# bbuchfink/diamond

Hardware: AMD Instinct MI355X
Metric: GCUPS + aligned queries/s, blastp --fast, 10000 queries vs 1000000-seq DB (seed stage + banded SW extension) (higher is better)
Workload: dtype int16

## Files before the change

### diamond_amd/csrc/ctx.h

```cpp
#pragma once
#include "tuning.h"
#include <hip/hip_runtime.h>
#include <chrono>
#include <cstdio>
#include <cstdlib>
#include <stdint.h>
#include <string>
#include <vector>
#include "../../include/diamond_hip.h"
#include "evalue.h"
#include "seed_ref_state.h"

namespace dmnd {

int fail(int code, const std::string& msg);

#define HIP_TRY(expr)                                                                                     \
	do {                                                                                                  \
		hipError_t e_ = (expr);                                                                           \
		if (e_ != hipSuccess)                                                                             \
			return ::dmnd::fail(DMND_E_DEVICE, std::string(#expr) + ": " + hipGetErrorString(e_));        \
	} while (0)

inline bool spin_sync()
// ... 121 lines not shown
	dmnd::DevBuf mask_lr, mask_pb, mask_scale, mask_pos, mask_ids, mask_soff, mask_long_ids, mask_long_soff, mask_long_pb, mask_long_scale;
	dmnd::DevBuf soft[2], motif_hit, motif_table;
	bool soft_valid[2] = { false, false };
	std::vector<uint64_t> motifs;
	bool own_motifs = false;
	double mask_ms = 0.0;
	double seed_ms[5] = { 0, 0, 0, 0, 0 };
	std::vector<dmnd::DevBuf> keep_trace;
	std::vector<dmnd_ctx*> aux;
	int8_t* pinned_cbs = nullptr; size_t pinned_cbs_cap = 0;
	double ext_stats[12] = { 0 };
	double ext_plan_stats[3] = { 0, 0, 0 };
	double host_ms[3] = { 0, 0, 0 };
	int comp_based_stats = 1;
	int query_contexts = 1;
	int max_target_seqs = 25;
	int frame_shift = 0;
	bool range_culling = false;
	double range_cover = 50.0;
	int fs_channels = 16;
	int max_hsps = 1;
	int global_ranking = 0;
	dmnd::DevBuf alt_targets;
	double top_percent = -1.0;
	double min_id = 0, query_cover = 0, subject_cover = 0, min_bit_score = 0;
	double approx_id = 0;
	dmnd_same_title_fn same_title = nullptr;
	void* same_title_user = nullptr;
	bool reuse_query_index = false;
	uint64_t query_generation = 0;
	uint64_t target_generation = 0;
	dmnd::SeedRefState seed_ref;
	int64_t seed_last_joined = -1;
	dmnd::DevBuf seed_ref_codes, seed_ref_lists, seed_ref_counts;
	void release_seed_ref_buffers() { seed_ref_codes.release(); seed_ref_lists.release(); seed_ref_counts.release(); }
	void release_seed_ref() { release_seed_ref_buffers(); seed_ref.seen = 0; seed_ref.key.clear(); }
	uint64_t cbs_generation = ~(uint64_t)0;
	std::string qindex_signature;
	std::vector<int32_t> source_lens;
	dmnd::DevBuf ext_source_lens;
	uint64_t source_lens_generation = ~(uint64_t)0;
	int ext_mode = -1;
	int band_mode_fast = 1;
	std::vector<unsigned long long> seed_trace;
	double ranking_block_letters = 2e9;
	dmnd::DevBuf seg_tables, seg_cls, seg_work, seg_handed, seg_ranges;
	bool seg_tables_ready = false;
	std::vector<int32_t> seg_last;
	bool seg_last_sorted = true;
	double seg_stats[4] = { 0, 0, 0, 0 };
};

struct KeptTrace {
	int arena = -1;
	bool kept = false;
	std::vector<int64_t> trace_off;
	std::vector<int32_t> P;
	std::vector<int32_t> score, end_i, end_j;
};
int dmnd_swipe_keep(dmnd_ctx* work, const dmnd_ctx* blocks, const dmnd_dp_target* items, int64_t n, int arena, dmnd_hsp* out, KeptTrace& kt);
int dmnd_traceback_kept(dmnd_ctx* work, const dmnd_ctx* blocks, const dmnd_dp_target* items, const KeptTrace& kt, const int64_t* src, int64_t n, dmnd_hsp* out);
namespace dmnd { struct SwipeEnd; }
namespace dmnd { int64_t sweep_rows_min_items(); }
int dmnd_sweep_classes(dmnd_ctx* work, const dmnd_ctx* blocks, const dmnd_dp_target* d_items, const uint32_t* class_count, const uint32_t* class_max_steps, int n_classes,
	const int32_t* order_dev, const int64_t* off_slot_dev, const int32_t* pairs_dev, const int64_t* off_item_dev, uint8_t* trace_dev, dmnd::SwipeEnd* ends_dev);
int dmnd_swipe_shared(dmnd_ctx* work, const dmnd_ctx* blocks, const dmnd_dp_target* items, int64_t n, int mode, uint32_t hsp_values,
	dmnd_hsp* out, uint8_t* transcript, int64_t transcript_cap, int64_t* transcript_used);
int dmnd_swipe_targets(dmnd_ctx* work, const dmnd_ctx* blocks, const int8_t* t, int64_t t_len, const dmnd_dp_target* items, int64_t n, int mode, uint32_t hsp_values,
// ... 13 lines not shown
```

### diamond_amd/csrc/seed_api.hip

```cpp
#include <hip/hip_runtime.h>
#include <algorithm>
#include <cstdlib>
#include <cmath>
#include <cstdio>
#include <cstring>
#include <string>
#include <sys/mman.h>
#include <thread>
#include <vector>
#include <chrono>
#include "ctx.h"
#include "seed_core.h"
#include "seed_kernels.h"

using namespace dmnd;

enum { SEED_CLASSES_LONG_DEFAULT = 1 };

static_assert(sizeof(dmnd_seed_params) == sizeof(SeedParams), "dmnd_seed_params must mirror dmnd::SeedParams");
static_assert(sizeof(dmnd_seed_hit) == 24, "dmnd_seed_hit layout");

extern "C" int dmnd_seed_params_fast(dmnd_seed_params* p, int threads)
{
	if (!p || threads < 1) return fail(DMND_E_ARG, "dmnd_seed_params_fast: bad argument");
// ... 541 lines not shown
		a.matched_count = c->counters.as<unsigned long long>() + sid;
		a.matched_cap = matched_cap;
		a.deferred = nullptr; a.deferred_count = c->counters.as<unsigned long long>() + S + 1; a.deferred_cap = 0;
		a.survivors = nullptr; a.survivor_count = c->counters.as<unsigned long long>() + S + 3; a.survivor_cap = 0;
		a.scored = nullptr; a.scored_count = c->counters.as<unsigned long long>() + S + 4;
		a.need_bits = c->seed_need.as<uint32_t>();
		a.e_key = nullptr; a.e_count = c->counters.as<unsigned long long>() + S + 2; a.e_n = 0;
		a.matrix = c->matrix.as<int8_t>();
		a.hits = c->seed_hits.as<dmnd_seed_hit>(); a.hit_count = c->counters.as<unsigned long long>() + S; a.hit_cap = 0;
		a.fused = fused ? 1 : 0;
		a.level2 = sp.shape_weight[sid] >= 10 ? 1 : 0;
		a.qfold = fused ? c->seed_qfold.as<uint8_t>() : nullptr;
		a.tfold = fused ? c->seed_tfold.as<uint8_t>() : nullptr;
		return a;
	};

	Timer tm(st);
	for (int i = 0; i < 5; ++i) c->seed_ms[i] = 0;
	lap("clears and query ids enqueued");
	SeedRefUse ref_use = SEED_REF_NONE;
	int slice_bits = -1;
	const int64_t ref_windows = seed_ref_windows(t_begin, t_end);
	{
		const int force = [] { const char* e = getenv("DMND_SEED_SLICES"); return e ? (atoi(e) != 0 ? 1 : 0) : -1; }();
		const uint64_t budget = [] { const char* e = getenv("DMND_SEED_SLICES_BUDGET_MB"); return (uint64_t)std::max<long long>(0, e ? atoll(e) : tuning().seed_slices_budget_mb); }() << 20;
		const int64_t min_letters = [] { const char* e = getenv("DMND_SEED_SLICES_MIN_LETTERS"); return e ? atoll(e) : tuning().seed_slices_min_letters; }();
		const uint32_t max_words = [] { const char* e = getenv("DMND_SEED_SLICE_WORDS"); return (uint32_t)std::min<long long>(SEED_SLICE_MAX_WORDS, std::max<long long>(64, e ? atoll(e) : SEED_SLICE_MAX_WORDS)); }();
		slice_bits = seed_slice_bits(bm1_words, slot_bits, max_words);
		const bool sparse_filter = (uint64_t)nq_pos * 4 <= bm1_words * 32;
		const bool eligible = !fused && !classes && nibble_shapes && sp.seed_encoding == SEED_SPACED && slice_bits >= 0 && ref_windows < ((int64_t)1 << 31)
			&& (force == 1 || (t_end - t_begin >= min_letters && sparse_filter && c->seed_last_joined <= tuning().seed_slices_max_joined));
		const int8_t* tseed = c->soft_valid[DMND_TARGET] ? c->soft[DMND_TARGET].as<int8_t>() : c->block[DMND_TARGET].as<int8_t>();
		bool drop = false;
		ref_use = seed_ref_decide(c->seed_ref, seed_ref_key_of(c->target_generation, tseed, t_begin, t_end, sp, slice_bits), force, eligible, seed_ref_cache_bytes(t_begin, t_end, S), budget, &drop);
		if (drop) c->release_seed_ref_buffers();
		if (ref_use == SEED_REF_BUILT) {
			const int64_t n_groups = seed_code_groups(t_begin, t_end);
			DevBuf route[2];
			auto exact = [](DevBuf& b, size_t bytes) {
				if (b.cap == bytes && b.own) return true;
				b.release();
				if (hipMalloc(&b.p, bytes) != hipSuccess) { b.p = nullptr; (void)hipGetLastError(); return false; }
				b.cap = bytes;
				return true;
			};
			bool ok = exact(c->seed_ref_codes, (size_t)n_groups * sizeof(uint64_t)) && c->seed_tflags.ensure((size_t)n_groups * sizeof(uint32_t)) == DMND_OK
				&& exact(c->seed_ref_lists, (size_t)S * (size_t)ref_windows * sizeof(uint32_t)) && exact(c->seed_ref_counts, (size_t)S * 64 * sizeof(uint32_t))
				&& exact(route[0], (size_t)ref_windows) && exact(route[1], (size_t)ref_windows);
			if (ok) {
				tm.start();
				hipError_t e = launch_seed_codes(sp, tseed, t_begin, t_end, c->seed_ref_codes.as<uint64_t>(), c->seed_tflags.as<uint32_t>(), nullptr, st);
				for (int sid = 0; sid < S && e == hipSuccess; ++sid)
					e = launch_seed_route(sp, sid, c->seed_ref_codes.as<uint64_t>(), c->seed_tflags.as<uint32_t>(), t_begin, t_end, slice_bits, route[0].as<uint8_t>(), route[1].as<uint8_t>(),
						c->seed_ref_lists.as<uint32_t>() + (size_t)sid * (size_t)ref_windows, c->seed_ref_counts.as<uint32_t>() + (size_t)sid * 64, &c->sort_tmp, &c->sort_tmp_bytes, st);
				tm.stop(c->seed_ms[0]);
				if (e == hipSuccess) e = sync_stream(st);
				if (e != hipSuccess) { route[0].release(); route[1].release(); c->release_seed_ref(); HIP_TRY(e); }
			}
			route[0].release(); route[1].release();
			seed_ref_built(c->seed_ref, ok);
			if (!ok) { c->release_seed_ref(); ref_use = SEED_REF_NONE; }
			lap("reference cache built");
		}
	}
	auto stream_shape = [&](const SeedArgs& a, int sid) -> hipError_t {
		if (ref_use == SEED_REF_NONE) return launch_seed_stream(a, sid, st);
		return launch_seed_stream_slices(a, sid, c->seed_ref_codes.as<uint64_t>(), c->seed_ref_lists.as<uint32_t>() + (size_t)sid * (size_t)ref_windows,
			c->seed_ref_counts.as<uint32_t>() + (size_t)sid * 64, slice_bits, st);
	};
	auto query_side = [&](const SeedArgs& a, int sid, bool build) -> int {
		if (build) {
			HIP_TRY(launch_seed_build(a, sid, c->seed_qlist.as<uint32_t>() + (size_t)(sid % SB) * nq_pos, c->seed_next.as<uint32_t>(), c->seed_qkeys.as<uint32_t>(),
				&c->sort_tmp, &c->sort_tmp_bytes, st));
		}
		else HIP_TRY(launch_seed_reset(a, sid, st));
		return DMND_OK;
	};
	if (c->soft_valid[DMND_QUERY]) {
		SeedArgs a = args_for(0, 0, 0);
		HIP_TRY(launch_seed_soft_time(a, st));
	}
	std::vector<unsigned long long> counts((size_t)S + 1, 0);
	unsigned long long n_pairs = 0;
	bool hits_done = false;
	char path[128] = "host";
	if (fused) {
		unsigned long long* ctr = c->counters.as<unsigned long long>();
		int64_t m_cap = seed_cap("DMND_SEED_MATCHED_CAP", std::max<int64_t>(std::max<int64_t>((int64_t)1 << 22, 4 * nq_pos), (int64_t)(std::min(c->matched_loc.cap / sizeof(int64_t), c->matched_slot.cap / sizeof(uint32_t)))));
		int64_t surv_cap = seed_cap("DMND_SEED_SURVIVOR_CAP", std::max<int64_t>((int64_t)1 << 20, (int64_t)(c->seed_survivors.cap / sizeof(SeedSurvivor))));
		int64_t hit_cap = seed_cap("DMND_SEED_HIT_CAP", std::max<int64_t>((int64_t)1 << 20, (int64_t)(c->seed_hits.cap / sizeof(dmnd_seed_hit))));
		if (int rc = c->seed_hits.ensure((size_t)hit_cap * sizeof(dmnd_seed_hit))) return rc;
		c->seed_trace.assign((size_t)2 * S, 0);
		int64_t hits_bound = 0;
		std::vector<unsigned long long> host_ctr((size_t)S + 4);
		hipStream_t sb = st;
		Timer tmb(sb);
		unsigned long long hits_seen = 0;
		bool hits_fresh = false;
		auto stage2 = [&](SeedArgs a, int sid, unsigned long long n, unsigned long long ns) -> int {
			HIP_TRY(hipSetDevice(c->device));
			if (hits_bound + (int64_t)ns > hit_cap) {
// ... 365 lines not shown
		if (int rc = c->sort_keys[1].ensure((size_t)n * sizeof(uint64_t))) return rc;
		if (int rc = c->sort_idx[0].ensure((size_t)n * sizeof(uint32_t))) return rc;
		if (int rc = c->sort_idx[1].ensure((size_t)n * sizeof(uint32_t))) return rc;
		uint64_t* keys[2] = { c->sort_keys[0].as<uint64_t>(), c->sort_keys[1].as<uint64_t>() };
		uint32_t* idx[2] = { c->sort_idx[0].as<uint32_t>(), c->sort_idx[1].as<uint32_t>() };
		auto bits_of = [](uint64_t v) { int b = 1; while (b < 64 && (v >> b) != 0) ++b; return b; };
		const std::vector<int64_t>& qlim = c->limits[DMND_QUERY];
		if (c->max_query_len_generation != c->query_generation || c->max_query_len <= 0) {
			int64_t m = 1;
			for (size_t i = 0; i + 1 < qlim.size(); ++i) m = std::max(m, qlim[i + 1] - qlim[i]);
			c->max_query_len = m; c->max_query_len_generation = c->query_generation;
		}
		HIP_TRY(sort_seed_hits(c->seed_hits.as<dmnd_seed_hit>(), c->seed_hits_sorted.as<dmnd_seed_hit>(), n, keys, idx, &c->sort_tmp, &c->sort_tmp_bytes, st,
			bits_of((uint64_t)std::max<size_t>(qlim.size(), 2) - 1), bits_of((uint64_t)c->block_len[DMND_TARGET]), bits_of((uint64_t)c->max_query_len), !sp.use_ungapped));
		HIP_TRY(sync_stream(st));
	}
	lap("hits sorted");
	if (phases) {
		unsigned long long t[8];
		HIP_TRY(copy_now(c->stream, t, c->counters.as<unsigned long long>() + S + 8, sizeof(t), hipMemcpyDeviceToHost));
		std::fprintf(stderr, "SEED_PHASES (ms of workgroup time, summed): start %.1f | windows %.1f | level 1 %.1f | table %.1f | light lists %.1f | heavy lists %.1f\n",
			t[0] / 1e5, t[1] / 1e5, t[2] / 1e5, t[3] / 1e5, t[4] / 1e5, t[5] / 1e5);
	}
	tm.collect();
	c->seed_ms[4] = c->seed_ms[0] + c->seed_ms[1] + c->seed_ms[2] + c->seed_ms[3];
	if (getenv("DMND_TRACE")) {
		std::fprintf(stderr, "dmnd_seed_search: %d shapes, %lld query positions, joined reference positions per shape:", S, (long long)nq_pos);
		for (int sid = 0; sid < S; ++sid) std::fprintf(stderr, " %llu", counts[sid]);
		std::fprintf(stderr, " | pairs %llu | Hamming survivors:", n_pairs);
		for (int sid = 0; sid < S && (size_t)sid < c->seed_trace.size(); ++sid) std::fprintf(stderr, " %llu", c->seed_trace[sid]);
		std::fprintf(stderr, " | deferred:");
		for (int sid = 0; sid < S && (size_t)(S + sid) < c->seed_trace.size(); ++sid) std::fprintf(stderr, " %llu", c->seed_trace[S + sid]);
		std::fprintf(stderr, " | hits %lld | ms index %.2f stream %.2f mask %.2f pairs %.2f | path: %s\n", (long long)c->n_seed_hits, c->seed_ms[0], c->seed_ms[1], c->seed_ms[2], c->seed_ms[3], path);
		const size_t held = c->seed_ref_codes.cap + c->seed_ref_lists.cap + c->seed_ref_counts.cap;
		if (ref_use == SEED_REF_NONE) std::fprintf(stderr, "dmnd_seed_search: stream: plain, reference cache: none, %zu bytes held\n", held);
		else std::fprintf(stderr, "dmnd_seed_search: stream: slices (%d x %g KB), reference cache: %s, %zu bytes held\n", 1 << slice_bits, (double)(bm1_words >> slice_bits) * 4 / 1024, ref_use == SEED_REF_BUILT ? "built" : "kept", held);
	}
	*n_hits = c->n_seed_hits;
	c->seed_last_hits = c->n_seed_hits;
	c->seed_last_joined = 0;
	for (int sid = 0; sid < S; ++sid) c->seed_last_joined += (int64_t)counts[sid];
	return DMND_OK;
}

extern "C" int64_t dmnd_seed_hit_count(const dmnd_ctx* c) { return c ? c->n_seed_hits : -1; }

extern "C" int dmnd_set_seed_hits_resident(dmnd_ctx* c, int on)
{
	if (!c) return fail(DMND_E_ARG, "dmnd_set_seed_hits_resident: ctx is NULL");
	c->seed_hits_stay = on != 0;
	return DMND_OK;
}

extern "C" int dmnd_seed_hits(dmnd_ctx* c, dmnd_seed_hit* out, int64_t cap)
{
	if (!c || (!out && c->n_seed_hits > 0)) return fail(DMND_E_ARG, "dmnd_seed_hits: NULL argument");
	if (cap < c->n_seed_hits) return fail(DMND_E_CAP, "dmnd_seed_hits: buffer too small");
	if (c->n_seed_hits == 0) return DMND_OK;
	if (c->seed_ret_hits == c->n_seed_hits && c->seed_ret_h.p) {
		std::memcpy(out, c->seed_ret_h.as<char>() + c->seed_ret_bytes_header, (size_t)c->n_seed_hits * sizeof(dmnd_seed_hit));
		return DMND_OK;
	}
	HIP_TRY(hipSetDevice(c->device));
	if (int rc = download_bytes(c, out, c->seed_hits_sorted.p, (size_t)c->n_seed_hits * sizeof(dmnd_seed_hit))) return rc;
	return DMND_OK;
}
```

### diamond_amd/csrc/seed_kernels.h

```cpp
#pragma once
#include <hip/hip_runtime.h>
#include <stdint.h>
#include "../../include/diamond_hip.h"
#include "seed_core.h"
#include "seed_chain.h"
#include "seed_slices_core.h"

namespace dmnd {

static const uint64_t SEED_EMPTY = ~0ull;
static const uint32_t LIST_END = 0xffffffffu;
enum : uint32_t { SLOT_JOINED = 1, SLOT_ERASED = 2, SLOT_LOWC = 8 };

struct SeedSlot { uint64_t key; uint32_t head; uint32_t flags; };

struct SeedDeferred { int64_t sloc; uint32_t slot, x; int32_t score, pad; };

struct SeedSurvivor { uint32_t slot, x; int64_t sloc; };

struct SeedScored { uint32_t slot, x; int64_t sloc; int32_t score, chunk; };

struct SeedArgs {
	SeedParams params;
	const int8_t* qdata; const int8_t* tdata;
// ... 26 lines not shown
	uint32_t* matched_slot; int64_t* matched_loc; unsigned long long* matched_count; int64_t matched_cap;
	SeedDeferred* deferred; unsigned long long* deferred_count; int64_t deferred_cap;
	SeedSurvivor* survivors; unsigned long long* survivor_count; int64_t survivor_cap;
	SeedScored* scored; unsigned long long* scored_count;
	uint32_t* need_bits;
	uint64_t* e_key; unsigned long long* e_count; int64_t e_n;
	const int8_t* matrix;
	dmnd_seed_hit* hits; unsigned long long* hit_count; int64_t hit_cap;
	const uint8_t* qfold;
	const uint8_t* tfold;
	int level2;
	int fused;
};

struct SeedClear {
	void* p[8]; uint64_t bytes[8]; uint32_t value[8];
	int n = 0;
	void add(void* ptr, uint64_t nbytes, uint32_t byte_value) { if (ptr && nbytes && n < 8) { p[n] = ptr; bytes[n] = nbytes; value[n] = byte_value; ++n; } }
};
hipError_t launch_seed_clear(const SeedClear& z, hipStream_t st);
hipError_t launch_seed_qid(const int64_t* limits, int64_t n_seqs, uint32_t* qid_of, hipStream_t st);
enum { SEED_NEED_FOLD_WORDS = 8192 };
hipError_t launch_seed_soft_time(const SeedArgs& a, hipStream_t st);
inline int64_t seed_build_work_words(int64_t n) { return 5 * n + 66; }
hipError_t launch_seed_build(const SeedArgs& a, int sid, uint32_t* qlist_out, uint32_t* work, uint32_t* sorted_top, void** tmp, size_t* tmp_bytes, hipStream_t st);
hipError_t launch_seed_reset(const SeedArgs& a, int sid, hipStream_t st);
hipError_t launch_seed_fold(const int8_t* data, int64_t n, uint8_t* out, hipStream_t st);
inline int64_t seed_code_groups(int64_t t_begin, int64_t t_end) { return (t_end - (t_begin & ~(int64_t)15) + 15) / 16 + 2; }
hipError_t launch_seed_codes(const SeedParams& c, const int8_t* tseed, int64_t t_begin, int64_t t_end, uint64_t* codes, uint32_t* flags, uint64_t* planes, hipStream_t st);
hipError_t launch_seed_stream(const SeedArgs& a, int sid, hipStream_t st, bool fused = false);
bool seed_stream_can_fuse(const SeedParams& c);
hipError_t launch_seed_route(const SeedParams& c, int sid, const uint64_t* codes, const uint32_t* flags, int64_t t_begin, int64_t t_end, int slice_bits,
	uint8_t* route, uint8_t* route_sorted, uint32_t* list, uint32_t* counts, void** tmp, size_t* tmp_bytes, hipStream_t st);
hipError_t launch_seed_stream_slices(const SeedArgs& a, int sid, const uint64_t* codes, const uint32_t* list, const uint32_t* counts, int slice_bits, hipStream_t st);
hipError_t launch_seed_mask(const SeedArgs& a, int sid, hipStream_t st, int64_t n_matched = -1);
hipError_t launch_seed_pairs(const SeedArgs& a, int sid, int64_t n_matched, hipStream_t st);
hipError_t launch_seed_pairs_tiled(const SeedArgs& a, int sid, int64_t n_matched, hipStream_t st);
hipError_t launch_seed_count_pairs(const SeedArgs& a, int64_t n_matched, unsigned long long* out, hipStream_t st);
hipError_t launch_seed_post(const SeedArgs& a, int sid, int64_t n_survivors, hipStream_t st, bool clear_scored = true);
hipError_t sort_matched_by_slot(const uint32_t* slot_in, uint32_t* slot_out, const int64_t* loc_in, int64_t* loc_out, int64_t n, int slot_bits,
	void** tmp, size_t* tmp_bytes, hipStream_t st);
hipError_t launch_seed_collect(const SeedArgs& a, int64_t n_matched, hipStream_t st);
hipError_t launch_seed_deferred(const SeedArgs& a, int sid, int64_t n_deferred, hipStream_t st);
hipError_t sort_keys_u64(const uint64_t* in, uint64_t* out, int64_t n, void** tmp, size_t* tmp_bytes, hipStream_t st);
hipError_t sort_seed_hits(const dmnd_seed_hit* hits, dmnd_seed_hit* out, int64_t n, uint64_t* keys[2], uint32_t* idx[2],
	void** tmp, size_t* tmp_bytes, hipStream_t st, int query_bits, int subject_bits, int off_bits, bool equal_scores = false);

struct SeedChain {
	unsigned long long* ctr;
	int S;
	int64_t matched_cap, survivor_cap, hit_cap, tiled_from;
};
hipError_t launch_seed_chain_streamed(const SeedChain& ch, int sid, hipStream_t st);
hipError_t launch_seed_chain_mask(const SeedArgs& a, const SeedChain& ch, int sid, hipStream_t st);
hipError_t launch_seed_chain_shape(const SeedArgs& a, const SeedChain& ch, int sid, hipStream_t st);
inline bool sort_seed_hits_one_key(int query_bits, int subject_bits, int off_bits) { return off_bits >= 1 && off_bits <= 24 && query_bits + subject_bits + off_bits <= 64; }
hipError_t launch_seed_chain_sort(const SeedChain& ch, bool sorted, const dmnd_seed_hit* hits, dmnd_seed_hit* out, int64_t sort_cap, uint64_t* keys[2], uint32_t* idx[2],
	void** tmp, size_t* tmp_bytes, hipStream_t st, int query_bits, int subject_bits, int off_bits, bool equal_scores, char* ret, int64_t ret_hits);

}
```

### diamond_amd/csrc/seed_kernels.hip

```cpp
#include <hip/hip_runtime.h>
#include <stdint.h>
#include "seed_core.h"
#include <algorithm>
#include <cstdlib>
#include <cstring>
#include <cstdio>
#include <rocprim/device/device_radix_sort.hpp>
#include <rocprim/iterator/counting_iterator.hpp>
#include <rocprim/iterator/transform_iterator.hpp>
#include <rocprim/iterator/transform_output_iterator.hpp>
#include <rocprim/device/device_scan.hpp>
#include "seed_kernels.h"

namespace dmnd {

struct SeedClearArgs { char* p[8]; uint64_t bytes[8]; uint64_t first_chunk[9]; uint32_t word[8]; int n; };
__global__ __launch_bounds__(256) void seed_clear_kernel(SeedClearArgs z)
{
	const uint64_t t = (uint64_t)blockIdx.x * blockDim.x + threadIdx.x;
	if (t >= z.first_chunk[8]) return;
	char* base = z.p[0];
	uint64_t bytes = z.bytes[0], first = 0;
	uint32_t w = z.word[0];
#pragma unroll
// ... 669 lines not shown
		}
		__syncthreads();
		PHASE_MARK(4);
		const unsigned n_heavy = hv_n < HEAVY ? hv_n : HEAVY;
		for (unsigned h = 0; h < n_heavy; ++h) {
			const unsigned k = hv_k[h];
			uint32_t count = st_count[k];
			if (count == 0xffffu) count = a.slot(st_slot[k]).flags >> 8;
			filter_list(st_slot[k], st_head[k], count, wg_base + st_loc[k], threadIdx.x, 256);
		}
		__syncthreads();
		PHASE_MARK(5);
		const unsigned n_sv = sv_n < SURV ? sv_n : SURV;
		if (n_sv) {
			if (threadIdx.x == 0) st_base = atomicAdd(a.survivor_count, (unsigned long long)n_sv);
			__syncthreads();
			for (unsigned k = threadIdx.x; k < n_sv; k += blockDim.x) {
				const unsigned long long idx = st_base + k;
				if (idx < (unsigned long long)a.survivor_cap) a.survivors[idx] = SeedSurvivor{ sv_slot[k], sv_x[k], wg_base + sv_loc[k] };
			}
			__syncthreads();
		}
	}
	const unsigned n_staged = st_n < STAGE ? st_n : STAGE;
	if (n_staged == 0) return;
	if (threadIdx.x == 0) st_base = atomicAdd(a.matched_count, (unsigned long long)n_staged);
	__syncthreads();
	for (unsigned k = threadIdx.x; k < n_staged; k += blockDim.x) {
		const unsigned long long idx = st_base + k;
		if (idx < (unsigned long long)a.matched_cap) { a.matched_slot[idx] = st_slot[k]; a.matched_loc[idx] = wg_base + st_loc[k]; }
	}
}

enum { SEED_SLICE_THREADS = 1024, SEED_SLICE_BATCH = 4, SEED_SLICE_QUEUE = 128, SEED_SLICE_STAGE = 32 };
__global__ __launch_bounds__(SEED_SLICE_THREADS) void seed_stream_slices_kernel(SeedArgs a, int64_t base, uint64_t care64, const uint64_t* __restrict__ codes,
	const uint32_t* __restrict__ list, const uint32_t* __restrict__ counts, int slice_bits, uint32_t slice_words)
{
	constexpr int B = SEED_SLICE_BATCH;
	constexpr unsigned WAVES = SEED_SLICE_THREADS / 64, QW = SEED_SLICE_QUEUE, ST = SEED_SLICE_STAGE;
	static_assert(QW >= 128, "a wavefront queues up to 63 + 64 positives before it probes 64");
	__shared__ uint32_t slice[SEED_SLICE_MAX_WORDS];
	__shared__ uint64_t q_key[WAVES][QW];
	__shared__ uint32_t q_off[WAVES][QW];
	__shared__ uint32_t st_slot[WAVES][ST], st_off[WAVES][ST];
	const unsigned s = blockIdx.x & ((1u << slice_bits) - 1), share = blockIdx.x >> slice_bits, shares = gridDim.x >> slice_bits;
	uint64_t begin = 0;
	for (unsigned i = 0; i < s; ++i) begin += counts[i];
	const uint64_t count = counts[s];
	const uint64_t lo = begin + count * share / shares, hi = begin + count * (share + 1) / shares;
	const uint32_t word0 = s * slice_words;
	for (uint32_t i = threadIdx.x; i < slice_words; i += blockDim.x) slice[i] = a.bitmap1[word0 + i];
	__syncthreads();
	const unsigned wave = threadIdx.x >> 6, lane = threadIdx.x & 63u;
	unsigned qn = 0, sn = 0;
	auto rank_in = [&](unsigned long long ballot) { return (unsigned)__builtin_amdgcn_mbcnt_hi((uint32_t)(ballot >> 32), __builtin_amdgcn_mbcnt_lo((uint32_t)ballot, 0u)); };
	auto wave_sync = [&]() { __builtin_amdgcn_fence(__ATOMIC_RELEASE, "wavefront"); __builtin_amdgcn_wave_barrier(); __builtin_amdgcn_fence(__ATOMIC_ACQUIRE, "wavefront"); };
	auto flush = [&]() {
		const unsigned n = sn < ST ? sn : ST;
		unsigned long long at = 0;
		if (lane == 0) at = atomicAdd(a.matched_count, (unsigned long long)n);
		at = ((unsigned long long)(uint32_t)__shfl((int)(at >> 32), 0) << 32) | (uint32_t)__shfl((int)(uint32_t)at, 0);
		wave_sync();
		if (lane < n && at + lane < (unsigned long long)a.matched_cap) { a.matched_slot[at + lane] = st_slot[wave][lane]; a.matched_loc[at + lane] = base + st_off[wave][lane]; }
		wave_sync();
		sn = 0;
	};
	auto probe = [&](bool active, uint64_t seed, uint32_t off) {
		bool found = false;
		uint64_t slot = 0;
		if (active) {
			const uint64_t hh = seed_hash(seed);
			if (!a.level2 || ((a.bitmap[a.bm2_index((uint32_t)hh, seed)] >> (uint32_t)(hh >> 59)) & 1u)) {
				slot = a.home(hh, seed);
				SeedSlot sl = a.slot(slot);
				uint32_t fl = 0;
				for (;;) {
					if (sl.key == SEED_EMPTY) break;
					if (sl.key == seed) { found = true; fl = sl.flags; break; }
					slot = (slot + 1) & a.slot_mask;
					sl = a.slot(slot);
				}
				if (found && !(fl & SLOT_JOINED)) a.slot(slot).flags = fl | SLOT_JOINED;
			}
		}
		const unsigned long long jb = __ballot(found);
		if (jb == 0) return;
		const unsigned k = sn + rank_in(jb);
		if (found) {
			if (k < ST) { st_slot[wave][k] = (uint32_t)slot; st_off[wave][k] = off; }
			else {
				const unsigned long long idx = atomicAdd(a.matched_count, 1ull);
				if (idx < (unsigned long long)a.matched_cap) { a.matched_slot[idx] = (uint32_t)slot; a.matched_loc[idx] = base + off; }
			}
		}
		sn += (unsigned)__builtin_popcountll(jb);
		if (sn >= ST / 2) flush();
	};
	const uint64_t stride = (uint64_t)B * blockDim.x;
	auto entries = [&](uint64_t k0, uint32_t* o) {
#pragma unroll
		for (int j = 0; j < B; ++j) {
			const uint64_t k = k0 + (uint64_t)j * blockDim.x + threadIdx.x;
			o[j] = k < hi ? list[k] : 0xffffffffu;
		}
	};
	auto nibbles = [&](const uint32_t* o, uint64_t* c0, uint64_t* c1) {
#pragma unroll
		for (int j = 0; j < B; ++j) {
			const uint32_t g = o[j] == 0xffffffffu ? 0u : o[j] >> 4;
			c0[j] = codes[g]; c1[j] = codes[g + 1];
		}
	};
	uint32_t off[B], off1[B], off2[B];
	uint64_t c0[B], c1[B], n0[B], n1[B];
	entries(lo, off);
	entries(lo + stride, off1);
	nibbles(off, c0, c1);
	for (uint64_t k0 = lo; k0 < hi; k0 += stride) {
		entries(k0 + 2 * stride, off2);
		nibbles(off1, n0, n1);
#pragma unroll
		for (int j = 0; j < B; ++j) {
			const int sh = (int)(off[j] & 15u) * 4;
			const uint64_t key = (sh == 0 ? c0[j] : (c0[j] >> sh) | (c1[j] << (64 - sh))) & care64;
			const uint32_t h = seed_hash_a(key);
			const uint32_t lw = a.bm1_index(h, key) - word0;
			const uint32_t bw = slice[lw < slice_words ? lw : 0u], need = bm1_bits(h, a.bitmap1_k3);
			const bool pass = off[j] != 0xffffffffu && (bw & need) == need;
			const unsigned long long pb = __ballot(pass);
			if (pb) {
				if (pass) { const unsigned k = qn + rank_in(pb); q_key[wave][k] = key; q_off[wave][k] = off[j]; }
				qn += (unsigned)__builtin_popcountll(pb);
				if (qn >= 64) {
					wave_sync();
					qn -= 64;
					const uint64_t seed = q_key[wave][qn + lane];
					const uint32_t o = q_off[wave][qn + lane];
					wave_sync();
					probe(true, seed, o);
				}
			}
		}
#pragma unroll
		for (int j = 0; j < B; ++j) { off[j] = off1[j]; off1[j] = off2[j]; c0[j] = n0[j]; c1[j] = n1[j]; }
	}
	wave_sync();
	{
		const bool active = lane < qn;
		const uint64_t seed = active ? q_key[wave][lane] : 0;
		const uint32_t o = active ? q_off[wave][lane] : 0;
		probe(active, seed, o);
	}
	if (sn) flush();
}

__global__ __launch_bounds__(256) void seed_route_kernel(const uint64_t* __restrict__ codes, const uint32_t* __restrict__ flags, int64_t base, int64_t n_groups, int64_t t_begin, int64_t t_end,
	int len, uint32_t care, uint64_t care64, int slice_bits, uint8_t* __restrict__ route, uint32_t* __restrict__ counts)
{
	__shared__ uint32_t hist[1 << SEED_SLICE_MAX_BITS];
	if (threadIdx.x < (1u << SEED_SLICE_MAX_BITS)) hist[threadIdx.x] = 0;
	__syncthreads();
	const int64_t g = (int64_t)blockIdx.x * blockDim.x + threadIdx.x;
	if (g < n_groups) {
		const int64_t p0 = base + 16 * g;
		uint8_t out[16];
		seed_route_group(codes[g], codes[g + 1], flags[g], flags[g + 1], t_begin - p0, t_end - p0, len, care, care64, slice_bits, out);
		uint32_t w[4] = { 0, 0, 0, 0 };
#pragma unroll
		for (int j = 0; j < 16; ++j) {
			w[j >> 2] |= (uint32_t)out[j] << ((j & 3) * 8);
			if (out[j] != SEED_ROUTE_NONE) atomicAdd(&hist[out[j]], 1u);
		}
		typedef uint32_t u32x4 __attribute__((ext_vector_type(4)));
		u32x4 v; v.x = w[0]; v.y = w[1]; v.z = w[2]; v.w = w[3];
		*reinterpret_cast<u32x4*>(route + 16 * g) = v;
	}
	__syncthreads();
	if (threadIdx.x < (1u << slice_bits) && hist[threadIdx.x]) atomicAdd(&counts[threadIdx.x], hist[threadIdx.x]);
}

__global__ void seed_mask_kernel(SeedArgs a, int sid)
{
	const uint64_t slot = (uint64_t)blockIdx.x * blockDim.x + threadIdx.x;
	if (slot > a.slot_mask) return;
	const SeedSlot sl = a.slot(slot);
// ... 873 lines not shown
static uint64_t care64_of(const SeedParams& c, int sid)
{
	uint64_t care64 = 0;
	for (int k = 0; k < c.shape_weight[sid]; ++k) care64 |= (uint64_t)15 << (4 * c.shape_pos[sid][k]);
	return care64;
}

hipError_t launch_seed_route(const SeedParams& c, int sid, const uint64_t* codes, const uint32_t* flags, int64_t t_begin, int64_t t_end, int slice_bits,
	uint8_t* route, uint8_t* route_sorted, uint32_t* list, uint32_t* counts, void** tmp, size_t* tmp_bytes, hipStream_t st)
{
	if (!seed_nibble_mode(c, sid) || c.seed_encoding != SEED_SPACED || slice_bits < 0 || slice_bits > SEED_SLICE_MAX_BITS) return hipErrorInvalidValue;
	const int64_t base = t_begin & ~(int64_t)15, n = seed_ref_windows(t_begin, t_end);
	if (n <= 0 || n >= ((int64_t)1 << 31)) return hipErrorInvalidValue;
	hipError_t e = hipMemsetAsync(counts, 0, ((size_t)1 << SEED_SLICE_MAX_BITS) * sizeof(uint32_t), st);
	if (e != hipSuccess) return e;
	hipLaunchKernelGGL(seed_route_kernel, dim3(blocks_for(n / 16, 256)), dim3(256), 0, st, codes, flags, base, n / 16, t_begin, t_end, (int)c.shape_len[sid], c.shape_mask[sid], care64_of(c, sid),
		slice_bits, route, counts);
	rocprim::counting_iterator<uint32_t> iota(0);
	size_t need = 0;
	e = rocprim::radix_sort_pairs(nullptr, need, route, route_sorted, iota, list, (size_t)n, 0, (unsigned)slice_bits + 1, st);
	if (e != hipSuccess) return e;
	if (need > *tmp_bytes) {
		if (*tmp) (void)hipFree(*tmp);
		*tmp = nullptr; *tmp_bytes = 0;
		e = hipMalloc(tmp, need);
		if (e != hipSuccess) return e;
		*tmp_bytes = need;
	}
	e = rocprim::radix_sort_pairs(*tmp, need, route, route_sorted, iota, list, (size_t)n, 0, (unsigned)slice_bits + 1, st);
	if (e != hipSuccess) return e;
	return hipGetLastError();
}

hipError_t launch_seed_stream_slices(const SeedArgs& a, int sid, const uint64_t* codes, const uint32_t* list, const uint32_t* counts, int slice_bits, hipStream_t st)
{
	const SeedParams& c = a.params;
	if (a.classes || a.fused || !seed_nibble_mode(c, sid) || c.seed_encoding != SEED_SPACED || slice_bits < 0 || slice_bits > SEED_SLICE_MAX_BITS) return hipErrorInvalidValue;
	if (a.bitmap1_words % (1u << slice_bits) != 0 || (a.bitmap1_words >> slice_bits) > (uint32_t)SEED_SLICE_MAX_WORDS || slice_bits > a.slot_bits) return hipErrorInvalidValue;
	int dev = 0, n_cus = 0;
	hipError_t e = hipGetDevice(&dev);
	if (e != hipSuccess) return e;
	e = hipDeviceGetAttribute(&n_cus, hipDeviceAttributeMultiprocessorCount, dev);
	if (e != hipSuccess) return e;
	n_cus = std::max(n_cus, 1);
	const unsigned slices = 1u << slice_bits, shares = std::max(1u, (unsigned)n_cus / slices);
	hipLaunchKernelGGL(seed_stream_slices_kernel, dim3(slices * shares), dim3(SEED_SLICE_THREADS), 0, st, a, a.t_begin & ~(int64_t)15, care64_of(c, sid), codes, list, counts, slice_bits,
		a.bitmap1_words >> slice_bits);
	return hipGetLastError();
}

hipError_t launch_seed_mask(const SeedArgs& a, int sid, hipStream_t st, int64_t n_matched)
{
	if (!a.fused && n_matched >= 0 && n_matched * 4 < (int64_t)a.slot_mask) {
		if (n_matched == 0) return hipSuccess;
		hipLaunchKernelGGL(seed_mask_joined_kernel<false>, dim3(blocks_for(n_matched, 256)), dim3(256), 0, st, a, sid, n_matched, SeedChain{});
		return hipGetLastError();
	}
	hipLaunchKernelGGL(seed_mask_kernel, dim3(blocks_for((int64_t)a.slot_mask + 1, 256)), dim3(256), 0, st, a, sid);
	return hipGetLastError();
}

hipError_t launch_seed_pairs(const SeedArgs& a, int sid, int64_t n_matched, hipStream_t st)
{
	if (n_matched == 0) return hipSuccess;
	hipLaunchKernelGGL(seed_pair_kernel<false>, dim3(blocks_for(n_matched, 128)), dim3(128), 0, st, a, sid, n_matched, SeedChain{});
	return hipGetLastError();
}

hipError_t launch_seed_pairs_tiled(const SeedArgs& a, int sid, int64_t n_matched, hipStream_t st)
{
	if (n_matched == 0) return hipSuccess;
	hipLaunchKernelGGL(seed_pair_tiled_kernel, dim3(blocks_for(n_matched, 256)), dim3(256), 0, st, a, sid, n_matched);
	return hipGetLastError();
}

hipError_t launch_seed_count_pairs(const SeedArgs& a, int64_t n_matched, unsigned long long* out, hipStream_t st)
{
	if (n_matched == 0) return hipSuccess;
	hipLaunchKernelGGL(seed_count_pairs_kernel, dim3(blocks_for(n_matched, 256)), dim3(256), 0, st, a, n_matched, out);
	return hipGetLastError();
// ... 269 lines not shown
```

### diamond_amd/csrc/seed_slices_core.h

```cpp
#pragma once
#include <stdint.h>
#include <string.h>
#include "seed_core.h"
#include "seed_ref_state.h"

namespace dmnd {

enum { SEED_SLICE_MAX_WORDS = 32768, SEED_SLICE_MAX_BITS = 6 };
enum : uint8_t { SEED_ROUTE_NONE = 0xff };

DMND_HD int seed_slice_bits(uint64_t words, int slot_bits, uint32_t max_words)
{
	if (max_words > (uint32_t)SEED_SLICE_MAX_WORDS) max_words = SEED_SLICE_MAX_WORDS;
	for (int b = 0; b <= SEED_SLICE_MAX_BITS; ++b) {
		if (words == 0 || words % ((uint64_t)1 << b) != 0) return -1;
		if ((words >> b) <= max_words) return b <= slot_bits ? b : -1;
	}
	return -1;
}

DMND_HD uint32_t seed_slice_of(uint32_t h, int slice_bits) { return slice_bits ? h >> (32 - slice_bits) : 0u; }

DMND_HD void seed_route_group(uint64_t c0, uint64_t c1, uint32_t f0, uint32_t f1, int64_t first, int64_t last, int len, uint32_t care, uint64_t care64, int slice_bits, uint8_t out[16])
{
	const uint32_t delim = (f0 & 0xffffu) | (f1 << 16), bad = (f0 >> 16) | (f1 & 0xffff0000u);
	const uint32_t span = (1u << len) - 1;
	for (int w = 0; w < 16; ++w) {
		const bool inside = w >= first && w < last && ((delim >> w) & span) == 0;
		const bool ok = inside && ((bad >> w) & care) == 0;
		const int sh = 4 * w;
		const uint64_t key = (sh == 0 ? c0 : (c0 >> sh) | (c1 << (64 - sh))) & care64;
		out[w] = ok ? (uint8_t)seed_slice_of(seed_hash_a(key), slice_bits) : (uint8_t)SEED_ROUTE_NONE;
	}
}

struct SeedRefKey {
	uint64_t generation;
	const void* tseed;
	int64_t t_begin, t_end;
	int32_t n_shapes, slice_bits, seed_encoding, reduction_size;
	int8_t reduction[32];
	int32_t shape_len[SEED_MAX_SHAPES];
	uint32_t shape_mask[SEED_MAX_SHAPES];
};

inline SeedRefKey seed_ref_key_of(uint64_t generation, const void* tseed, int64_t t_begin, int64_t t_end, const SeedParams& sp, int slice_bits)
{
	SeedRefKey k;
	memset(&k, 0, sizeof(k));
	k.generation = generation; k.tseed = tseed; k.t_begin = t_begin; k.t_end = t_end;
	k.n_shapes = sp.n_shapes; k.slice_bits = slice_bits; k.seed_encoding = sp.seed_encoding; k.reduction_size = sp.reduction_size;
	memcpy(k.reduction, sp.reduction, sizeof(k.reduction));
	for (int i = 0; i < sp.n_shapes && i < SEED_MAX_SHAPES; ++i) { k.shape_len[i] = sp.shape_len[i]; k.shape_mask[i] = sp.shape_mask[i]; }
	return k;
}

inline std::string seed_ref_key_bytes(const SeedRefKey& k) { return std::string(reinterpret_cast<const char*>(&k), sizeof(SeedRefKey)); }

inline int64_t seed_ref_windows(int64_t t_begin, int64_t t_end) { return ((t_end - (t_begin & ~(int64_t)15) + 15) / 16) * 16; }
inline uint64_t seed_ref_cache_bytes(int64_t t_begin, int64_t t_end, int n_shapes)
{
	const uint64_t n = (uint64_t)seed_ref_windows(t_begin, t_end);
	return (uint64_t)n_shapes * (n * sizeof(uint32_t) + 64 * sizeof(uint32_t)) + (n / 16 + 2) * sizeof(uint64_t);
}

enum SeedRefUse { SEED_REF_NONE = 0, SEED_REF_BUILT = 1, SEED_REF_KEPT = 2 };
inline SeedRefUse seed_ref_decide(SeedRefState& s, const SeedRefKey& k, int force, bool eligible, uint64_t bytes, uint64_t budget, bool* drop)
{
	const std::string kb = seed_ref_key_bytes(k);
	const bool same = s.seen != 0 && s.key == kb;
	*drop = s.seen == 2 && !same;
	if (!same) { s.seen = 0; }
	if (force == 0 || !eligible || bytes > budget) {
		return SEED_REF_NONE;
	}
	if (same && s.seen == 2) return SEED_REF_KEPT;
	if (force == 1 || same) { s.key = kb; return SEED_REF_BUILT; }
	s.key = kb; s.seen = 1;
	return SEED_REF_NONE;
}
inline void seed_ref_built(SeedRefState& s, bool ok) { s.seen = ok ? 2 : 0; }

}
```

Baseline: 192.1.

## Precompute cached reference seed hashes and stream them with deep vector prefetch

When the reference slice cache is built, a new kernel computes and stores the seed hash for every routed list entry. The slice streaming kernel then reads precomputed hashes and offsets with 16-byte nontemporal loads, prefetched four rounds deep, instead of gathering codes and rehashing per entry. Codes are fetched only for entries that pass the bitmap filter, and the shared-memory key queue is dropped. The cost is an extra hash array per shape, which counts against the cache budget and may disable the cache in more cases, plus extra build-time work.

```diff
diff --git a/diamond_amd/csrc/ctx.h b/diamond_amd/csrc/ctx.h
--- a/diamond_amd/csrc/ctx.h
+++ b/diamond_amd/csrc/ctx.h
@@ -177,8 +177,8 @@
 	uint64_t target_generation = 0;
 	dmnd::SeedRefState seed_ref;
 	int64_t seed_last_joined = -1;
-	dmnd::DevBuf seed_ref_codes, seed_ref_lists, seed_ref_counts;
-	void release_seed_ref_buffers() { seed_ref_codes.release(); seed_ref_lists.release(); seed_ref_counts.release(); }
+	dmnd::DevBuf seed_ref_codes, seed_ref_lists, seed_ref_hashes, seed_ref_counts;
+	void release_seed_ref_buffers() { seed_ref_codes.release(); seed_ref_lists.release(); seed_ref_hashes.release(); seed_ref_counts.release(); }
 	void release_seed_ref() { release_seed_ref_buffers(); seed_ref.seen = 0; seed_ref.key.clear(); }
 	uint64_t cbs_generation = ~(uint64_t)0;
 	std::string qindex_signature;
diff --git a/diamond_amd/csrc/seed_api.hip b/diamond_amd/csrc/seed_api.hip
--- a/diamond_amd/csrc/seed_api.hip
+++ b/diamond_amd/csrc/seed_api.hip
@@ -597,7 +597,7 @@
 			&& (force == 1 || (t_end - t_begin >= min_letters && sparse_filter && c->seed_last_joined <= tuning().seed_slices_max_joined));
 		const int8_t* tseed = c->soft_valid[DMND_TARGET] ? c->soft[DMND_TARGET].as<int8_t>() : c->block[DMND_TARGET].as<int8_t>();
 		bool drop = false;
-		ref_use = seed_ref_decide(c->seed_ref, seed_ref_key_of(c->target_generation, tseed, t_begin, t_end, sp, slice_bits), force, eligible, seed_ref_cache_bytes(t_begin, t_end, S), budget, &drop);
+		ref_use = seed_ref_decide(c->seed_ref, seed_ref_key_of(c->target_generation, tseed, t_begin, t_end, sp, slice_bits), force, eligible, seed_ref_cache_bytes(t_begin, t_end, S) + seed_ref_hash_bytes(t_begin, t_end, S), budget, &drop);
 		if (drop) c->release_seed_ref_buffers();
 		if (ref_use == SEED_REF_BUILT) {
 			const int64_t n_groups = seed_code_groups(t_begin, t_end);
@@ -610,14 +610,18 @@
 				return true;
 			};
 			bool ok = exact(c->seed_ref_codes, (size_t)n_groups * sizeof(uint64_t)) && c->seed_tflags.ensure((size_t)n_groups * sizeof(uint32_t)) == DMND_OK
-				&& exact(c->seed_ref_lists, (size_t)S * (size_t)ref_windows * sizeof(uint32_t)) && exact(c->seed_ref_counts, (size_t)S * 64 * sizeof(uint32_t))
+				&& exact(c->seed_ref_lists, (size_t)S * (size_t)ref_windows * sizeof(uint32_t)) && exact(c->seed_ref_hashes, (size_t)S * (size_t)ref_windows * sizeof(uint32_t))
+				&& exact(c->seed_ref_counts, (size_t)S * 64 * sizeof(uint32_t))
 				&& exact(route[0], (size_t)ref_windows) && exact(route[1], (size_t)ref_windows);
 			if (ok) {
 				tm.start();
 				hipError_t e = launch_seed_codes(sp, tseed, t_begin, t_end, c->seed_ref_codes.as<uint64_t>(), c->seed_tflags.as<uint32_t>(), nullptr, st);
-				for (int sid = 0; sid < S && e == hipSuccess; ++sid)
+				for (int sid = 0; sid < S && e == hipSuccess; ++sid) {
+					uint32_t* list = c->seed_ref_lists.as<uint32_t>() + (size_t)sid * (size_t)ref_windows;
 					e = launch_seed_route(sp, sid, c->seed_ref_codes.as<uint64_t>(), c->seed_tflags.as<uint32_t>(), t_begin, t_end, slice_bits, route[0].as<uint8_t>(), route[1].as<uint8_t>(),
-						c->seed_ref_lists.as<uint32_t>() + (size_t)sid * (size_t)ref_windows, c->seed_ref_counts.as<uint32_t>() + (size_t)sid * 64, &c->sort_tmp, &c->sort_tmp_bytes, st);
+						list, c->seed_ref_counts.as<uint32_t>() + (size_t)sid * 64, &c->sort_tmp, &c->sort_tmp_bytes, st);
+					if (e == hipSuccess) e = launch_seed_ref_hashes(sp, sid, c->seed_ref_codes.as<uint64_t>(), list, t_begin, t_end, c->seed_ref_hashes.as<uint32_t>() + (size_t)sid * (size_t)ref_windows, st);
+				}
 				tm.stop(c->seed_ms[0]);
 				if (e == hipSuccess) e = sync_stream(st);
 				if (e != hipSuccess) { route[0].release(); route[1].release(); c->release_seed_ref(); HIP_TRY(e); }
@@ -631,7 +635,7 @@
 	auto stream_shape = [&](const SeedArgs& a, int sid) -> hipError_t {
 		if (ref_use == SEED_REF_NONE) return launch_seed_stream(a, sid, st);
 		return launch_seed_stream_slices(a, sid, c->seed_ref_codes.as<uint64_t>(), c->seed_ref_lists.as<uint32_t>() + (size_t)sid * (size_t)ref_windows,
-			c->seed_ref_counts.as<uint32_t>() + (size_t)sid * 64, slice_bits, st);
+			c->seed_ref_hashes.as<uint32_t>() + (size_t)sid * (size_t)ref_windows, c->seed_ref_counts.as<uint32_t>() + (size_t)sid * 64, slice_bits, st);
 	};
 	auto query_side = [&](const SeedArgs& a, int sid, bool build) -> int {
 		if (build) {
@@ -1063,7 +1067,7 @@
 		std::fprintf(stderr, " | deferred:");
 		for (int sid = 0; sid < S && (size_t)(S + sid) < c->seed_trace.size(); ++sid) std::fprintf(stderr, " %llu", c->seed_trace[S + sid]);
 		std::fprintf(stderr, " | hits %lld | ms index %.2f stream %.2f mask %.2f pairs %.2f | path: %s\n", (long long)c->n_seed_hits, c->seed_ms[0], c->seed_ms[1], c->seed_ms[2], c->seed_ms[3], path);
-		const size_t held = c->seed_ref_codes.cap + c->seed_ref_lists.cap + c->seed_ref_counts.cap;
+		const size_t held = c->seed_ref_codes.cap + c->seed_ref_lists.cap + c->seed_ref_hashes.cap + c->seed_ref_counts.cap;
 		if (ref_use == SEED_REF_NONE) std::fprintf(stderr, "dmnd_seed_search: stream: plain, reference cache: none, %zu bytes held\n", held);
 		else std::fprintf(stderr, "dmnd_seed_search: stream: slices (%d x %g KB), reference cache: %s, %zu bytes held\n", 1 << slice_bits, (double)(bm1_words >> slice_bits) * 4 / 1024, ref_use == SEED_REF_BUILT ? "built" : "kept", held);
 	}
diff --git a/diamond_amd/csrc/seed_kernels.h b/diamond_amd/csrc/seed_kernels.h
--- a/diamond_amd/csrc/seed_kernels.h
+++ b/diamond_amd/csrc/seed_kernels.h
@@ -82,7 +82,8 @@
 bool seed_stream_can_fuse(const SeedParams& c);
 hipError_t launch_seed_route(const SeedParams& c, int sid, const uint64_t* codes, const uint32_t* flags, int64_t t_begin, int64_t t_end, int slice_bits,
 	uint8_t* route, uint8_t* route_sorted, uint32_t* list, uint32_t* counts, void** tmp, size_t* tmp_bytes, hipStream_t st);
-hipError_t launch_seed_stream_slices(const SeedArgs& a, int sid, const uint64_t* codes, const uint32_t* list, const uint32_t* counts, int slice_bits, hipStream_t st);
+hipError_t launch_seed_ref_hashes(const SeedParams& c, int sid, const uint64_t* codes, const uint32_t* list, int64_t t_begin, int64_t t_end, uint32_t* hashes, hipStream_t st);
+hipError_t launch_seed_stream_slices(const SeedArgs& a, int sid, const uint64_t* codes, const uint32_t* list, const uint32_t* hashes, const uint32_t* counts, int slice_bits, hipStream_t st);
 hipError_t launch_seed_mask(const SeedArgs& a, int sid, hipStream_t st, int64_t n_matched = -1);
 hipError_t launch_seed_pairs(const SeedArgs& a, int sid, int64_t n_matched, hipStream_t st);
 hipError_t launch_seed_pairs_tiled(const SeedArgs& a, int sid, int64_t n_matched, hipStream_t st);
diff --git a/diamond_amd/csrc/seed_kernels.hip b/diamond_amd/csrc/seed_kernels.hip
--- a/diamond_amd/csrc/seed_kernels.hip
+++ b/diamond_amd/csrc/seed_kernels.hip
@@ -725,15 +725,14 @@
 	}
 }
 
-enum { SEED_SLICE_THREADS = 1024, SEED_SLICE_BATCH = 4, SEED_SLICE_QUEUE = 128, SEED_SLICE_STAGE = 32 };
+enum { SEED_SLICE_THREADS = 1024, SEED_SLICE_BATCH = 4, SEED_SLICE_DEPTH = 4, SEED_SLICE_QUEUE = 128, SEED_SLICE_STAGE = 32 };
 __global__ __launch_bounds__(SEED_SLICE_THREADS) void seed_stream_slices_kernel(SeedArgs a, int64_t base, uint64_t care64, const uint64_t* __restrict__ codes,
-	const uint32_t* __restrict__ list, const uint32_t* __restrict__ counts, int slice_bits, uint32_t slice_words)
-{
-	constexpr int B = SEED_SLICE_BATCH;
+	const uint32_t* __restrict__ list, const uint32_t* __restrict__ hashes, const uint32_t* __restrict__ counts, int slice_bits, uint32_t slice_words)
+{
+	constexpr int B = SEED_SLICE_BATCH, DEPTH = SEED_SLICE_DEPTH;
 	constexpr unsigned WAVES = SEED_SLICE_THREADS / 64, QW = SEED_SLICE_QUEUE, ST = SEED_SLICE_STAGE;
 	static_assert(QW >= 128, "a wavefront queues up to 63 + 64 positives before it probes 64");
 	__shared__ uint32_t slice[SEED_SLICE_MAX_WORDS];
-	__shared__ uint64_t q_key[WAVES][QW];
 	__shared__ uint32_t q_off[WAVES][QW];
 	__shared__ uint32_t st_slot[WAVES][ST], st_off[WAVES][ST];
 	const unsigned s = blockIdx.x & ((1u << slice_bits) - 1), share = blockIdx.x >> slice_bits, shares = gridDim.x >> slice_bits;
@@ -789,61 +788,53 @@
 		sn += (unsigned)__builtin_popcountll(jb);
 		if (sn >= ST / 2) flush();
 	};
-	const uint64_t stride = (uint64_t)B * blockDim.x;
-	auto entries = [&](uint64_t k0, uint32_t* o) {
-#pragma unroll
-		for (int j = 0; j < B; ++j) {
-			const uint64_t k = k0 + (uint64_t)j * blockDim.x + threadIdx.x;
-			o[j] = k < hi ? list[k] : 0xffffffffu;
-		}
+	auto probe_queued = [&](bool active, uint32_t e) {
+		const uint32_t off = active ? e : 0u;
+		const uint64_t seed = seed_window_key(codes[off >> 4], codes[(off >> 4) + 1], off & 15u, care64);
+		probe(active, seed, off);
 	};
-	auto nibbles = [&](const uint32_t* o, uint64_t* c0, uint64_t* c1) {
-#pragma unroll
-		for (int j = 0; j < B; ++j) {
-			const uint32_t g = o[j] == 0xffffffffu ? 0u : o[j] >> 4;
-			c0[j] = codes[g]; c1[j] = codes[g + 1];
+	typedef uint32_t u32x4 __attribute__((ext_vector_type(4)));
+	static_assert(B == 4, "one 16-byte load per round");
+	const uint64_t stride = (uint64_t)B * blockDim.x, first = (lo & ~(uint64_t)(B - 1)) + (uint64_t)B * threadIdx.x;
+	u32x4 hv[DEPTH], ov[DEPTH];
+	auto request = [&](uint64_t k, u32x4& h, u32x4& o) {
+		h = 0; o = 0;
+		if (k < hi) {
+			h = __builtin_nontemporal_load(reinterpret_cast<const u32x4*>(hashes + k));
+			o = __builtin_nontemporal_load(reinterpret_cast<const u32x4*>(list + k));
 		}
 	};
-	uint32_t off[B], off1[B], off2[B];
-	uint64_t c0[B], c1[B], n0[B], n1[B];
-	entries(lo, off);
-	entries(lo + stride, off1);
-	nibbles(off, c0, c1);
-	for (uint64_t k0 = lo; k0 < hi; k0 += stride) {
-		entries(k0 + 2 * stride, off2);
-		nibbles(off1, n0, n1);
-#pragma unroll
-		for (int j = 0; j < B; ++j) {
-			const int sh = (int)(off[j] & 15u) * 4;
-			const uint64_t key = (sh == 0 ? c0[j] : (c0[j] >> sh) | (c1[j] << (64 - sh))) & care64;
-			const uint32_t h = seed_hash_a(key);
-			const uint32_t lw = a.bm1_index(h, key) - word0;
-			const uint32_t bw = slice[lw < slice_words ? lw : 0u], need = bm1_bits(h, a.bitmap1_k3);
-			const bool pass = off[j] != 0xffffffffu && (bw & need) == need;
-			const unsigned long long pb = __ballot(pass);
-			if (pb) {
-				if (pass) { const unsigned k = qn + rank_in(pb); q_key[wave][k] = key; q_off[wave][k] = off[j]; }
-				qn += (unsigned)__builtin_popcountll(pb);
-				if (qn >= 64) {
-					wave_sync();
-					qn -= 64;
-					const uint64_t seed = q_key[wave][qn + lane];
-					const uint32_t o = q_off[wave][qn + lane];
-					wave_sync();
-					probe(true, seed, o);
+#pragma unroll
+	for (int d = 0; d < DEPTH; ++d) request(first + (uint64_t)d * stride, hv[d], ov[d]);
+	for (uint64_t k0 = first; k0 < hi + (uint64_t)B * threadIdx.x; k0 += (uint64_t)DEPTH * stride) {
+#pragma unroll
+		for (int d = 0; d < DEPTH; ++d) {
+			const u32x4 h4 = hv[d], o4 = ov[d];
+			const uint64_t k = k0 + (uint64_t)d * stride;
+			request(k + (uint64_t)DEPTH * stride, hv[d], ov[d]);
+#pragma unroll
+			for (int j = 0; j < B; ++j) {
+				const uint32_t h = h4[j];
+				const uint32_t lw = seed_slice_word(h, a.bm1_hmask, a.bitmap1_words) - word0;
+				const uint32_t bw = slice[lw < slice_words ? lw : 0u], need = bm1_bits(h, a.bitmap1_k3);
+				const bool pass = k + j >= lo && k + j < hi && (bw & need) == need;
+				const unsigned long long pb = __ballot(pass);
+				if (pb) {
+					if (pass) q_off[wave][qn + rank_in(pb)] = o4[j];
+					qn += (unsigned)__builtin_popcountll(pb);
+					if (qn >= 64) {
+						wave_sync();
+						qn -= 64;
+						const uint32_t e = q_off[wave][qn + lane];
+						wave_sync();
+						probe_queued(true, e);
+					}
 				}
 			}
 		}
-#pragma unroll
-		for (int j = 0; j < B; ++j) { off[j] = off1[j]; off1[j] = off2[j]; c0[j] = n0[j]; c1[j] = n1[j]; }
 	}
 	wave_sync();
-	{
-		const bool active = lane < qn;
-		const uint64_t seed = active ? q_key[wave][lane] : 0;
-		const uint32_t o = active ? q_off[wave][lane] : 0;
-		probe(active, seed, o);
-	}
+	probe_queued(lane < qn, lane < qn ? q_off[wave][lane] : 0u);
 	if (sn) flush();
 }
 
@@ -1783,7 +1774,7 @@
 	return hipGetLastError();
 }
 
-hipError_t launch_seed_stream_slices(const SeedArgs& a, int sid, const uint64_t* codes, const uint32_t* list, const uint32_t* counts, int slice_bits, hipStream_t st)
+hipError_t launch_seed_stream_slices(const SeedArgs& a, int sid, const uint64_t* codes, const uint32_t* list, const uint32_t* hashes, const uint32_t* counts, int slice_bits, hipStream_t st)
 {
 	const SeedParams& c = a.params;
 	if (a.classes || a.fused || !seed_nibble_mode(c, sid) || c.seed_encoding != SEED_SPACED || slice_bits < 0 || slice_bits > SEED_SLICE_MAX_BITS) return hipErrorInvalidValue;
@@ -1795,8 +1786,23 @@
 	if (e != hipSuccess) return e;
 	n_cus = std::max(n_cus, 1);
 	const unsigned slices = 1u << slice_bits, shares = std::max(1u, (unsigned)n_cus / slices);
-	hipLaunchKernelGGL(seed_stream_slices_kernel, dim3(slices * shares), dim3(SEED_SLICE_THREADS), 0, st, a, a.t_begin & ~(int64_t)15, care64_of(c, sid), codes, list, counts, slice_bits,
-		a.bitmap1_words >> slice_bits);
+	hipLaunchKernelGGL(seed_stream_slices_kernel, dim3(slices * shares), dim3(SEED_SLICE_THREADS), 0, st, a, a.t_begin & ~(int64_t)15, care64_of(c, sid), codes, list, hashes,
+		counts, slice_bits, a.bitmap1_words >> slice_bits);
+	return hipGetLastError();
+}
+
+__global__ __launch_bounds__(256) void seed_ref_hash_kernel(const uint64_t* __restrict__ codes, const uint32_t* __restrict__ list, int64_t n, uint64_t care64, uint32_t* __restrict__ hashes)
+{
+	const int64_t k = (int64_t)blockIdx.x * blockDim.x + threadIdx.x;
+	if (k < n) hashes[k] = seed_ref_hash_entry(codes, list[k], care64);
+}
+
+hipError_t launch_seed_ref_hashes(const SeedParams& c, int sid, const uint64_t* codes, const uint32_t* list, int64_t t_begin, int64_t t_end, uint32_t* hashes, hipStream_t st)
+{
+	if (!seed_nibble_mode(c, sid) || c.seed_encoding != SEED_SPACED) return hipErrorInvalidValue;
+	const int64_t n = seed_ref_windows(t_begin, t_end);
+	if (n <= 0 || n >= ((int64_t)1 << 31)) return hipErrorInvalidValue;
+	hipLaunchKernelGGL(seed_ref_hash_kernel, dim3(blocks_for(n, 256)), dim3(256), 0, st, codes, list, n, care64_of(c, sid), hashes);
 	return hipGetLastError();
 }
 
diff --git a/diamond_amd/csrc/seed_slices_core.h b/diamond_amd/csrc/seed_slices_core.h
--- a/diamond_amd/csrc/seed_slices_core.h
+++ b/diamond_amd/csrc/seed_slices_core.h
@@ -21,6 +21,17 @@
 
 DMND_HD uint32_t seed_slice_of(uint32_t h, int slice_bits) { return slice_bits ? h >> (32 - slice_bits) : 0u; }
 
+DMND_HD uint32_t seed_slice_word(uint32_t h, uint32_t hmask, uint32_t words) { return bm1_word(h & hmask, words); }
+DMND_HD uint64_t seed_window_key(uint64_t c0, uint64_t c1, uint32_t at, uint64_t care64)
+{
+	const int sh = 4 * (int)at;
+	return (sh == 0 ? c0 : (c0 >> sh) | (c1 << (64 - sh))) & care64;
+}
+DMND_HD uint32_t seed_ref_hash_entry(const uint64_t* codes, uint32_t off, uint64_t care64)
+{
+	return seed_hash_a(seed_window_key(codes[off >> 4], codes[(off >> 4) + 1], off & 15u, care64));
+}
+
 DMND_HD void seed_route_group(uint64_t c0, uint64_t c1, uint32_t f0, uint32_t f1, int64_t first, int64_t last, int len, uint32_t care, uint64_t care64, int slice_bits, uint8_t out[16])
 {
 	const uint32_t delim = (f0 & 0xffffu) | (f1 << 16), bad = (f0 >> 16) | (f1 & 0xffff0000u);
@@ -28,8 +39,7 @@
 	for (int w = 0; w < 16; ++w) {
 		const bool inside = w >= first && w < last && ((delim >> w) & span) == 0;
 		const bool ok = inside && ((bad >> w) & care) == 0;
-		const int sh = 4 * w;
-		const uint64_t key = (sh == 0 ? c0 : (c0 >> sh) | (c1 << (64 - sh))) & care64;
+		const uint64_t key = seed_window_key(c0, c1, (uint32_t)w, care64);
 		out[w] = ok ? (uint8_t)seed_slice_of(seed_hash_a(key), slice_bits) : (uint8_t)SEED_ROUTE_NONE;
 	}
 }
@@ -63,6 +73,10 @@
 	const uint64_t n = (uint64_t)seed_ref_windows(t_begin, t_end);
 	return (uint64_t)n_shapes * (n * sizeof(uint32_t) + 64 * sizeof(uint32_t)) + (n / 16 + 2) * sizeof(uint64_t);
 }
+inline uint64_t seed_ref_hash_bytes(int64_t t_begin, int64_t t_end, int n_shapes)
+{
+	return (uint64_t)n_shapes * (uint64_t)seed_ref_windows(t_begin, t_end) * sizeof(uint32_t);
+}
 
 enum SeedRefUse { SEED_REF_NONE = 0, SEED_REF_BUILT = 1, SEED_REF_KEPT = 2 };
 inline SeedRefUse seed_ref_decide(SeedRefState& s, const SeedRefKey& k, int force, bool eligible, uint64_t bytes, uint64_t budget, bool* drop)
```

Result: faster. 214.2 (median of 6 runs) (+11.5%).
